# bschrag620/PyRad

Measured on AMD Instinct MI355X. Metric: line*gridpoint evals/sec (whole job), higher is better.
Workload: dtype f64

## Files before the change

### pyrad_amd/csrc/lbl_api.hip

```cpp
#include "../../include/pyrad_hip.h"
#include "lbl_device.h"

#include <algorithm>
#include <chrono>
#include <cmath>
#include <cstdarg>
#include <cstdio>
#include <cstdlib>
#include <cstring>
#include <memory>
#include <mutex>
#include <new>
#include <stdexcept>
#include <string>
#include <type_traits>
#include <vector>


using namespace lbl;
namespace lbl {
void comm_quiesce(lbl_ctx* ctx);
void comm_forget(lbl_ctx* ctx);
}

// ... 17 lines not shown
    DeviceArena cidx;
    DeviceArena work;
    DeviceArena jobs;
    DeviceArena counts;
    DeviceArena bal;
    DeviceArena red;
    DeviceArena zeros;
    size_t zeros_set = 0;
    void* host_stage = nullptr;
    size_t host_stage_cap = 0;
    size_t host_stage_head = 0;
    hipEvent_t stage_ev[2] = {nullptr, nullptr};
    bool stage_ev_set[2] = {false, false};
    struct DescSlot { std::vector<char> bytes; void* dptr = nullptr; size_t cap = 0; };
    DescSlot desc_cache[4];
    int desc_next = 0;
    std::vector<char> desc_build;
    int last_jobs = 0;
    int last_blocks_per_job = 0;
    std::vector<int> last_list_blocks;
    int accum_variant = 5;
    int accum_R = 0;
    int accum_LS = 0;
    int gauss_run = 0;
    int bal_workers[9] = {0, 0, 0, 0, 0, 0, 0, 0, 0};
    struct Schedule {
        std::vector<uint64_t> key; int2* d_list; int total; int32_t* d_tabs; std::vector<size_t> tab_off;
        int xcd_tol = 3;
        int sr_chunks = 1;
        int launch_total = 0;
        int xcd_pack = 1;
        void* d_block = nullptr;
        bool pending = false;
        int R = 0, spans_per_tile = 0, total_spans = 0, xcd_chunks = 32;
        long long far_reach = 0;
        double cost_near = 0, cost_edge = 0, cost_far = 0, cost_fixed = 0;
        std::vector<int32_t> span_first, tile_first;
        int32_t* d_src = nullptr;
        std::vector<size_t> src_off;
        bool merge_pending = false;
    };
    std::vector<std::unique_ptr<Schedule>> schedules;
    int accuracy = 0;
    int sweep_ieee = 0;
    int sched_build = 1;
    DeviceArena sched;
// ... 374 lines not shown
} LBL_GUARD_END(ctx)

extern "C" int lbl_profile_read(lbl_ctx* ctx, int kind, int64_t* launches, double* total_ms) try {
    if (!ctx || !launches || !total_ms) return fail(ctx, LBL_ERR_BAD_ARG, "NULL argument");
    if (kind < 0 || kind >= kProfileKinds) return fail(ctx, LBL_ERR_BAD_ARG, "kind out of range");
    HIP_TRY(ctx, hipStreamSynchronize(ctx->stream));
    double tot = 0.0;
    for (auto& p : ctx->ev_rec[kind]) {
        float ms = 0.f;
        HIP_TRY(ctx, hipEventElapsedTime(&ms, p.first, p.second));
        tot += ms;
    }
    *launches = (int64_t)ctx->ev_rec[kind].size();
    *total_ms = tot;
    return LBL_OK;
} LBL_GUARD_END(ctx)

namespace lbl {
void* comm_prof_begin(lbl_ctx* ctx) { return (void*)prof_begin(ctx, PROF_GATHER); }
void comm_prof_end(lbl_ctx* ctx, void* start) { prof_end(ctx, PROF_GATHER, (hipEvent_t)start); }
}

static uint64_t option_state(const lbl_ctx* c) {
    const long long v[] = {c->accum_variant, c->accum_R, c->accum_LS, c->gauss_run, c->lpt, c->tile_order, c->skew, c->skew_R, c->skew_LS, c->xcd_chunks, c->xcd_pack, c->xcd_tol, c->far_min_H,
                           c->ablate, c->accuracy, c->sweep_ieee, c->sched_build, c->no_fuse ? 1 : 0,
                           c->bal_workers[1], c->bal_workers[2], c->bal_workers[4], c->bal_workers[8]};
    uint64_t h = 1469598103934665603ull;
    for (long long x : v) { h ^= (uint64_t)x; h *= 1099511628211ull; }
    return h;
}
static int set_option_value(lbl_ctx* ctx, const char* key, int value);

extern "C" int lbl_set_option(lbl_ctx* ctx, const char* key, int value) try {
    if (!ctx || !key) return fail(ctx, LBL_ERR_BAD_ARG, "NULL argument");
    const uint64_t before = option_state(ctx);
    const int rc = set_option_value(ctx, key, value);
    if (option_state(ctx) != before) ctx->epoch++;
    return rc;
} LBL_GUARD_END(ctx)

static int set_option_value(lbl_ctx* ctx, const char* key, int value) {
    if (!strcmp(key, "accum_variant")) {
#ifdef LBL_DIAG
        if (value < 0 || value > 5) return fail(ctx, LBL_ERR_BAD_ARG, "accum_variant must be 0..5");
#else
        if (!(value == 0 || value == 3 || value == 5))
            return fail(ctx, LBL_ERR_BAD_ARG, "accum_variant must be 0, 3 or 5 (1, 2 and 4 are superseded comparison kernels: diagnostic builds only)");
// ... 19 lines not shown
    } else if (!strcmp(key, "accum_skew")) {
        if (value < 0 || value > 2) return fail(ctx, LBL_ERR_BAD_ARG, "accum_skew must be 0, 1 or 2");
        ctx->skew = value;
    } else if (!strcmp(key, "accum_skew_points_per_lane")) {
        if (!(value == 1 || value == 2 || value == 4 || value == 8))
            return fail(ctx, LBL_ERR_BAD_ARG, "accum_skew_points_per_lane must be 1, 2, 4 or 8");
        ctx->skew_R = value;
    } else if (!strcmp(key, "accum_xcd_chunks")) {
        if (value < 0 || value > 64) return fail(ctx, LBL_ERR_BAD_ARG, "accum_xcd_chunks must be 0 (auto: 10..32 by the workgroup count) .. 64");
        ctx->xcd_chunks = value;
    } else if (!strcmp(key, "accum_xcd_tolerance")) {
        if (value < -1 || value > 15) return fail(ctx, LBL_ERR_BAD_ARG, "accum_xcd_tolerance must be -1 (off) .. 15 percent");
        ctx->xcd_tol = value;
    } else if (!strcmp(key, "accum_xcd_pack")) {
        if (value < 0 || value > 3) return fail(ctx, LBL_ERR_BAD_ARG, "accum_xcd_pack must be 0..3");
        ctx->xcd_pack = value;
    } else if (!strcmp(key, "accum_skew_line_split")) {
        if (!(value == 0 || value == 1 || value == 2 || value == 4))
            return fail(ctx, LBL_ERR_BAD_ARG, "accum_skew_line_split must be 0 (auto), 1, 2 or 4");
        ctx->skew_LS = value;
    } else if (!strcmp(key, "accum_gauss_run")) {
        if (value != 0 && value != 16 && value != 32) return fail(ctx, LBL_ERR_BAD_ARG, "accum_gauss_run must be 0 (auto), 16 or 32");
        ctx->gauss_run = value;
    } else if (!strcmp(key, "accum_far_min_window")) {
        if (value < 0) return fail(ctx, LBL_ERR_BAD_ARG, "accum_far_min_window must be >= 0");
        ctx->far_min_H = value;
#ifdef LBL_DIAG
    } else if (!strcmp(key, "debug_ablate")) {
        ctx->ablate = value;
#endif
    } else if (!strcmp(key, "accuracy")) {
        if (value < 0 || value > 1) return fail(ctx, LBL_ERR_BAD_ARG, "accuracy must be 0 (exact) or 1 (budget: 1e-9)");
        ctx->accuracy = value;
    } else if (!strcmp(key, "sweep_ieee_divisions")) {
        if (value < 0 || value > 1) return fail(ctx, LBL_ERR_BAD_ARG, "sweep_ieee_divisions must be 0 or 1");
        ctx->sweep_ieee = value;
    } else if (!strcmp(key, "schedule_build")) {
        if (value < 0 || value > 1) return fail(ctx, LBL_ERR_BAD_ARG, "schedule_build must be 0 (host) or 1 (device)");
        ctx->sched_build = value;
    } else if (!strcmp(key, "layer_step_fused")) {
        if (value < 0 || value > 1) return fail(ctx, LBL_ERR_BAD_ARG, "layer_step_fused must be 0 or 1");
        ctx->no_fuse = value == 0;
    } else if (!strcmp(key, "debug_throw")) {
        if (value == 1) throw std::bad_alloc();
        if (value == 2) throw std::runtime_error("debug_throw");
        if (value == 3) { std::vector<double> v; v.reserve(v.max_size() + 1); }
// ... 818 lines not shown
                              sc->far_reach, sc->cost_near, sc->cost_edge, sc->cost_far, sc->cost_fixed,
                              ctx->n_cu > 0 ? ctx->n_cu : 256, sc->d_tabs, (char*)ctx->sched.ptr + jobs_bytes, sc->d_list, ctx->stream,
                              sc->xcd_chunks, sc->xcd_pack != 0, sc->sr_chunks, sc->xcd_tol, sc->xcd_pack == 2 ? 1 : sc->xcd_pack == 3 ? 0 : -1);
        HIP_TRY(ctx, hipGetLastError());
        sc->pending = false;
    }
    if (ctx->chain_pred && !ctx->capturing) HIP_TRY(ctx, hipStreamWaitEvent(ctx->stream, ctx->chain_pred->accum_done, 0));
    for (size_t gi = 0; gi < groups.size(); ++gi) {
        const Group& g = groups[gi];
        ev = prof_begin(ctx, PROF_ACCUM);
        if (balanced) {
            const size_t S = (size_t)group_spans[gi];
            char* base = (char*)ctx->bal.ptr + bal_off[gi];
            SpanRec* spans = (SpanRec*)base;
            unsigned long long* prefix = (unsigned long long*)(base + S * sizeof(SpanRec));
            unsigned int* cnts = (unsigned int*)(base + S * sizeof(SpanRec) + (S + 1) * sizeof(unsigned long long));
            double* slab = (double*)(base + ((S * sizeof(SpanRec) + S * sizeof(unsigned int) + (S + 1) * sizeof(unsigned long long) + 255) & ~(size_t)255));
            launch_accumulate_balanced(da + g.first, g.count, (int)S, g.R, group_workers[gi], spans, cnts, prefix, slab,
                                       ctx->stream);
        } else if (g.variant == 6) {
            launch_accumulate_skew(da + g.first, g.count, g.max_tiles, g.R, g.worklist, g.total_tiles, ctx->stream, g.LS);
        } else {
            launch_accumulate(da + g.first, g.count, g.max_tiles, g.R, g.LS, g.variant, g.worklist, g.total_tiles,
                              ctx->stream, ctx->accuracy, g.grun);
        }
        prof_end(ctx, PROF_ACCUM, ev);
        HIP_TRY(ctx, hipGetLastError());
    }
    if (ctx->accum_done && !ctx->capturing) HIP_TRY(ctx, hipEventRecord(ctx->accum_done, ctx->stream));
    for (int j = 0; j < n_jobs; ++j) {
        if (!needs_regrid(grid[j])) continue;
        ev = prof_begin(ctx, PROF_REGRID);
        launch_regrid((const double*)ctx->work.ptr + work_off[j], grid[j].n_work, out_dev[j], grid[j].n_base,
                      grid[j].range_min, grid[j].range_max, ctx->stream);
        prof_end(ctx, PROF_REGRID, ev);
        HIP_TRY(ctx, hipGetLastError());
    }
    return LBL_OK;
}

extern "C" int lbl_schedule_export(lbl_ctx* ctx, int k, int32_t* list, int64_t list_cap, int32_t* tabs, int64_t tabs_cap,
                                   int64_t* n_items, int64_t* n_tab_ints, int32_t* built_on_device) try {
    if (!ctx || !n_items || !n_tab_ints) return fail(ctx, LBL_ERR_BAD_ARG, "NULL argument");
    if (k < 0 || (size_t)k >= ctx->schedules.size()) return fail(ctx, LBL_ERR_BAD_ARG, "no such schedule (the cache holds %d)", (int)ctx->schedules.size());
    const lbl_ctx::Schedule& S = *ctx->schedules[ctx->schedules.size() - 1 - (size_t)k];
    if (S.pending) return fail(ctx, LBL_ERR_STATE, "the schedule has not been built yet (no accumulate batch has used it)");
    HIP_TRY(ctx, hipStreamSynchronize(ctx->stream));
// ... 867 lines not shown
```

### pyrad_amd/csrc/lbl_device.h

```cpp
#pragma once
#include <hip/hip_runtime.h>
#include <stdint.h>
#include "lbl_launch_shapes.h"

namespace lbl {

constexpr double kB = 1.38064852E-23;
constexpr double cLight = 299792458.0;
constexpr double hPlanck = 6.62607004e-34;
constexpr double kPi = 3.141592653589793;
constexpr double kInvPi = 0.3183098861837907;
constexpr double kInvSqrtPi = 0.5641895835477563;
constexpr double t0 = 296.0;
constexpr double p0 = 1013.25;
constexpr double avo = 6.022140857E23;

struct __attribute__((aligned(32))) HotRec {
    double cf;
    double a2;
    double KL;
    int32_t dgi;
    int32_t flags;
};
struct __attribute__((aligned(32))) ColdRec {
// ... 198 lines not shown
    double table_half, table_rdx;
    long long n_channels;
    int32_t n_rows, n_table;
    int32_t chunk, pad;
};
void launch_ils_convolve(const IlsArgs* d_args, int shape, int n_rows, long long n_channels, hipStream_t s);

struct ColumnArgs {
    const double* trans[kMaxLayers];
    double layer_T[kMaxLayers];
    double r_layer_T[kMaxLayers];
    double pbkT[kMaxLayers], pbk_surface;
    double r_surface_T;
    int32_t n_layers;
    double start, stop, step, pa, pb, surface_T;
    const double* I_in; double* I_out;
    long long n;
    long long first, count;
};

void launch_line_prep(const PrepJob* d_jobs, int n_jobs, int max_lines, hipStream_t s);
void launch_line_quantities(const PrepJob* d_job, int n_lines, long long* index, double* lhw, double* ghw, double* intensity,
                            int32_t* regime, hipStream_t s);
void launch_accumulate(const AccumJob* d_jobs, int n_jobs, int max_tiles, int R, int LS, int variant,
                       const int2* worklist, int total_tiles, hipStream_t s, int budget = 0, int gauss_run = 16);
void launch_accumulate_skew(const AccumJob* d_jobs, int n_jobs, int max_tiles, int R, const int2* worklist, int total_tiles,
                            hipStream_t s, int LS = 1);
void accumulate_far_field_params(int R, int* far_half_spans, double* far_cost, int budget = 0);
int balanced_workers(int R, int n_cu);
void launch_accumulate_balanced(const AccumJob* d_jobs, int n_jobs, int total_spans, int R, int n_workers,
                                SpanRec* spans, unsigned int* counts, unsigned long long* prefix, double* slab,
                                hipStream_t s);
void launch_regrid(const double* work, long long n_work, double* out, long long n_base, double start, double stop,
                   hipStream_t s);
void launch_layer_sweep(const SweepArgs& a, hipStream_t s);
void launch_column_step(const ColumnStepArgs* d_args, long long first, long long count, hipStream_t s, int budget = 0, int kfold = 0);
void launch_column_sweep(const ColumnArgs* d_args, long long n, hipStream_t s, int budget = 0);
void launch_planck(double* out, long long n, double start, double stop, double T, double rT, double pa, double pb, hipStream_t s);
void launch_band_integral(const double* y, long long n, double* partial, double* result, hipStream_t s);
struct SumArgs { const double* in[kMaxIso]; int32_t n_in; double* out; long long n; };
void launch_sum(const SumArgs& a, hipStream_t s);
constexpr int kMaxRanks = 64;
struct CompactArgs { const double* gathered; double* out; long long slot; long long first[kMaxRanks]; long long count[kMaxRanks]; int32_t world; };
void launch_gather_compact(const CompactArgs& a, long long max_count, hipStream_t s);
void launch_optical(const double* trans, long long n, int kind, double* out, hipStream_t s);
void launch_line_survey(const double* nu, const double* sw, int n_lines, double range_min, double resolution,
                        double* out, long long n_base, hipStream_t s);

// ... 2 lines not shown
```

### pyrad_amd/csrc/lbl_kernels.hip

```cpp
#include "lbl_device.h"
#include "lbl_launch_shapes.h"
#include <cstdlib>
#include <type_traits>

namespace lbl {

#ifdef LBL_DIAG
#define LBL_ABLATE(obj, bit) (((obj).ablate & (bit)) != 0)
#else
#define LBL_ABLATE(obj, bit) false
#endif

__device__ __forceinline__ int uniform_i32(int v) { return __builtin_amdgcn_readfirstlane(v); }

typedef const double __attribute__((address_space(4)))* ConstF64;
typedef const int32_t __attribute__((address_space(4)))* ConstI32;

struct Rec {
    double cf, a2, KL, KG, b, q2;
    int32_t ci, dgi, flags;
};

__device__ __forceinline__ Rec load_rec_scalar(const HotRec* hot, const ColdRec* cold, int i, bool want_cold) {
    ConstF64 h = (ConstF64)(unsigned long long)hot + (long long)i * 4;
// ... 396 lines not shown
            const double t = K * S.D[k];
            S.N[k] = fma(S.N[k], den, t);
            S.D[k] *= den;
        }
        if (++S.cnt == S.every) S.flush();
    }
}

template <int R, bool MASKED, int DIV, int GM>
__device__ __forceinline__ void process_lines_scalar(const HotRec* hot, const ColdRec* cold, int i0, int i1, double x0,
                                                     int wlo, int whi, double Hf, WaveAcc<R>& S) {
    for (int i = i0; i < i1; ++i) {
        Rec r = load_rec_scalar(hot, cold, i, false);
        const double d0 = x0 - r.cf;
        lorentz_term<R, MASKED, DIV>(r.a2, r.KL, r.flags, d0, Hf, S);
        const int dist = max(0, max(r.ci - whi, wlo - r.ci));
        if (dist < r.dgi) {
            r = load_rec_scalar(hot, cold, i, true);
            gauss_term<R, GM>(r.KG, r.b, r.q2 >= 0.0, d0, Hf, r.q2, S.acc);
        }
    }
}

__device__ __forceinline__ void wave_line_ranges(const int32_t* __restrict__ cidx, int n_lines, int wlo, int whi, int H,
                                                 int lane, int& iA, int& iB, int& iC, int& iD) {
    const long long tA = (long long)wlo - H, tB = (long long)whi - H;
    const long long tC = (long long)wlo + H + 1, tD = (long long)whi + H + 1;
    const int q = lane >> 4, jj = lane & 15;
    const long long tgt = q == 0 ? tA : q == 1 ? tB : q == 2 ? tC : tD;
    const unsigned long long gmask = 0xFFFFull << (q * 16);
    int lo = 0, hi = n_lines;
    while (__any(hi > lo)) {
        const long long len = (long long)hi - lo;
        const int pos = lo + (int)(((long long)(jj + 1) * len) / 17);
        const bool below = (len > 0) && ((long long)cidx[len > 0 ? pos : 0] < tgt);
        const int k = __popcll(__ballot(below) & gmask);
        if (len > 0) {
            const int p_k = lo + (int)(((long long)(k + 1) * len) / 17);
            const int p_km1 = lo + (int)(((long long)k * len) / 17);
            const int new_lo = k > 0 ? p_km1 + 1 : lo;
            const int new_hi = k < 16 ? p_k : hi;
            lo = new_lo; hi = new_hi;
        }
    }
    iA = __builtin_amdgcn_readlane(lo, 0);
    iB = __builtin_amdgcn_readlane(lo, 16);
    iC = __builtin_amdgcn_readlane(lo, 32);
    iD = __builtin_amdgcn_readlane(lo, 48);
    if (tB >= tC) { iB = iD; iC = iD; }
}

__device__ __forceinline__ void wave_line_ranges_far(const int32_t* __restrict__ cidx, int n_lines, int wlo, int whi, int H,
                                                     long long fl, long long fr, int lane, int& iA, int& iB, int& iC,
                                                     int& iD, int& iF1, int& iF2, int& iN1, int& iN2, long long nl, long long nr) {
    const long long tA = (long long)wlo - H, tB = (long long)whi - H;
    const long long tC = (long long)wlo + H + 1, tD = (long long)whi + H + 1;
    const int q = lane >> 3, jj = lane & 7;
    const long long tgt = q == 0 ? tA : q == 1 ? tB : q == 2 ? tC : q == 3 ? tD : q == 4 ? fl + 1 : q == 5 ? fr : q == 6 ? nl + 1 : nr;
    const unsigned long long gmask = 0xFFull << (q * 8);
    int lo = 0, hi = n_lines;
    while (__any(hi > lo)) {
        const long long len = (long long)hi - lo;
        const int pos = lo + (int)(((long long)(jj + 1) * len) / 9);
        const bool below = (len > 0) && ((long long)cidx[len > 0 ? pos : 0] < tgt);
        const int k = __popcll(__ballot(below) & gmask);
        if (len > 0) {
            const int p_k = lo + (int)(((long long)(k + 1) * len) / 9);
            const int p_km1 = lo + (int)(((long long)k * len) / 9);
            const int new_lo = k > 0 ? p_km1 + 1 : lo;
            const int new_hi = k < 8 ? p_k : hi;
            lo = new_lo; hi = new_hi;
// ... 318 lines not shown
constexpr int FF_NT_MID = 38;
template <int NT> struct LorentzNear { static constexpr int value = NT == FF_NT_MID ? FF_MID : FarThreshold<NT>::value; };

template <int CTRL>
__device__ __forceinline__ double dpp_move_f64(double v) {
    int lo = __double2loint(v), hi = __double2hiint(v);
    lo = __builtin_amdgcn_update_dpp(0, lo, CTRL, 0xf, 0xf, true);
    hi = __builtin_amdgcn_update_dpp(0, hi, CTRL, 0xf, 0xf, true);
    return __hiloint2double(hi, lo);
}

__device__ __forceinline__ double readlane_f64(double v, int l) {
    return __hiloint2double(__builtin_amdgcn_readlane(__double2hiint(v), l), __builtin_amdgcn_readlane(__double2loint(v), l));
}

__device__ __forceinline__ double wave_sum_f64(double v) {
    v += dpp_move_f64<0xB1>(v);
    v += dpp_move_f64<0x4E>(v);
    v += dpp_move_f64<0x141>(v);
    v += dpp_move_f64<0x140>(v);
    return (readlane_f64(v, 0) + readlane_f64(v, 16)) + (readlane_f64(v, 32) + readlane_f64(v, 48));
}

template <int NT>
__device__ __forceinline__ void wave_sum_rows(double (&C)[NT], double* scratch, int lane) {
    const int wr = lane + (lane >> 3);
    const int rd = (lane >> 3) * 72 + (lane & 7) * 9;
#pragma unroll
    for (int base = 0; base < NT; base += 8) {
        __builtin_amdgcn_wave_barrier();
#pragma unroll
        for (int n = 0; n < 8; ++n)
            if (base + n < NT) scratch[n * 72 + wr] = C[base + n];
        __builtin_amdgcn_fence(__ATOMIC_RELEASE, "wavefront");
        __builtin_amdgcn_wave_barrier();
        double t = 0.0;
        if (base + (lane >> 3) < NT) {
            const double* seg = scratch + rd;
            t = ((seg[0] + seg[1]) + (seg[2] + seg[3])) + ((seg[4] + seg[5]) + (seg[6] + seg[7]));
        }
        t += dpp_move_f64<0xB1>(t);
        t += dpp_move_f64<0x4E>(t);
        t += dpp_move_f64<0x141>(t);
#pragma unroll
        for (int n = 0; n < 8; ++n)
            if (base + n < NT) C[base + n] = readlane_f64(t, n * 8);
    }
    __builtin_amdgcn_wave_barrier();
}

template <int NT> struct FarTerms {
    static constexpr bool exact = NT == FF_NT || NT == FF_NT_MID, budget = NT == FF_NT_BUDGET;
    static constexpr int t4 = budget ? 18 : (NT == FF_NT_MID ? FF_NT : NT);
    static constexpr int t8 = exact ? 20 : (budget ? 12 : NT);
    static constexpr int t16 = exact ? 15 : (budget ? 9 : NT);
    static constexpr int t32 = exact ? 12 : (budget ? 7 : NT);
};

template <int N0, int N1, int NT>
__device__ __forceinline__ void series_terms(double al, double bp, double& qa, double& qb, double (&C)[NT]) {
#pragma unroll
    for (int n = N0; n < N1; ++n) {
        const double qn = fma(al, qb, -(bp * qa));
        C[n] += qn;
        if ((n & 1) == 1) asm volatile("" : "+v"(C[n]));
        qa = qb; qb = qn;
    }
}

template <int R, int NT>
__device__ __forceinline__ void far_field_lines(const HotRec* hot, const ColdRec* cold, int m0, int m1, int stride,
                                                double xc, int wlo, int whi, double x0, double Hf, double* lh, double* lc,
                                                int lane, double (&C)[NT], WaveAcc<R>& S, int gx_lo = 0, int gx_hi = 0) {
    typedef double v2f64 __attribute__((ext_vector_type(2)));
    typedef const v2f64 __attribute__((address_space(1)))* GlobalF64x2;
    const GlobalF64x2 gh = (GlobalF64x2)(unsigned long long)hot;
    const GlobalF64x2 gc = (GlobalF64x2)(unsigned long long)cold;
    const double hh = 32.0 * R;
    v2f64 h0 = {0, 1}, h1 = {0, 0};
    if (m0 + lane < m1) {
        const long long r = (long long)(m0 + lane) * 2;
        h0 = gh[r]; h1 = gh[r + 1];
    }
    for (int c0 = m0; c0 < m1; c0 += stride) {
        const bool valid = c0 + lane < m1;
        const v2f64 w0 = h0, w1 = h1;
        if (c0 + stride + lane < m1) {
            const long long r = (long long)(c0 + stride + lane) * 2;
            h0 = gh[r]; h1 = gh[r + 1];
        }
        const int ci = (int)w0.x;
        const int dgi = __double2loint(w1.y), fl = __double2hiint(w1.y);
        const bool gauss = valid && max(0, max(ci - whi, wlo - ci)) < dgi && !(c0 + lane >= gx_lo && c0 + lane < gx_hi);
        const unsigned long long gmask = __ballot(gauss);
        if (gmask) {
            const unsigned long long emask = __ballot((fl & REC_NO_RECUR) != 0);
            v2f64 c0v = {0, 0}, c1v = {0, 0};
            if (gauss) {
                const long long r = (long long)(c0 + lane) * 2;
                c0v = gc[r]; c1v = gc[r + 1];
            }
            __builtin_amdgcn_wave_barrier();
            reinterpret_cast<v2f64*>(lh)[lane * 2] = w0;
            reinterpret_cast<v2f64*>(lh)[lane * 2 + 1] = w1;
            reinterpret_cast<v2f64*>(lc)[lane * 2] = c0v;
            reinterpret_cast<v2f64*>(lc)[lane * 2 + 1] = c1v;
            __builtin_amdgcn_fence(__ATOMIC_RELEASE, "wavefront");
            __builtin_amdgcn_wave_barrier();
            double unused[16];
            chunk_extras<R, 0>(lh, lc, gmask, emask, 0ull, ~0ull, x0, Hf, S, 0ull, 0.0, lane, unused);
            __builtin_amdgcn_wave_barrier();
        }
        const double dl = w0.x - xc;
        const double sq = fma(dl, dl, w0.y);
        double be = __builtin_amdgcn_rcp(sq);
        be = fma(fma(-sq, be, 1.0), be, be);
        be = fma(fma(-sq, be, 1.0), be, be);
        const double al = (dl * (2.0 * hh)) * be;
        const double bp = (hh * hh) * be;
        double qa = (valid ? w1.x : 0.0) * be;
        C[0] += qa;
        double qb = al * qa;
        C[1] += qb;
        const int nv = min(64, m1 - c0);
        const int ca = __builtin_amdgcn_readlane(ci, 0), cb = __builtin_amdgcn_readlane(ci, nv - 1);
        const int dmin2 = min(abs(2 * (ca - wlo) - (64 * R - 1)), abs(2 * (cb - wlo) - (64 * R - 1)));
        typedef FarTerms<NT> FT;
        series_terms<2, FT::t32, NT>(al, bp, qa, qb, C);
        if (dmin2 < 2 * 32 * 32 * R) {
            series_terms<FT::t32, FT::t16, NT>(al, bp, qa, qb, C);
            if (dmin2 < 2 * 16 * 32 * R) {
                series_terms<FT::t16, FT::t8, NT>(al, bp, qa, qb, C);
                if (dmin2 < 2 * 8 * 32 * R) {
                    series_terms<FT::t8, FT::t4, NT>(al, bp, qa, qb, C);
                    if (FT::t4 < NT && dmin2 < 2 * 4 * 32 * R) series_terms<FT::t4, NT, NT>(al, bp, qa, qb, C);
                }
            }
        }
    }
}

template <int R> struct SkewChunk { static constexpr int value = R >= 8 ? 80 : 112; };

__device__ __forceinline__ unsigned int dpp_max_u32(unsigned int v, unsigned int moved) { return v > moved ? v : moved; }

__device__ __forceinline__ unsigned int wave_prefix_max_u32(unsigned int v) {
    v = dpp_max_u32(v, (unsigned int)__builtin_amdgcn_update_dpp(0, (int)v, 0x111, 0xf, 0xf, false));
    v = dpp_max_u32(v, (unsigned int)__builtin_amdgcn_update_dpp(0, (int)v, 0x112, 0xf, 0xf, false));
    v = dpp_max_u32(v, (unsigned int)__builtin_amdgcn_update_dpp(0, (int)v, 0x114, 0xf, 0xf, false));
    v = dpp_max_u32(v, (unsigned int)__builtin_amdgcn_update_dpp(0, (int)v, 0x118, 0xf, 0xf, false));
    v = dpp_max_u32(v, (unsigned int)__builtin_amdgcn_update_dpp(0, (int)v, 0x142, 0xa, 0xf, false));
    v = dpp_max_u32(v, (unsigned int)__builtin_amdgcn_update_dpp(0, (int)v, 0x143, 0xc, 0xf, false));
    return v;
}

template <int R>
__device__ __forceinline__ void skew_counts(const unsigned int* __restrict__ cnt, int lane, int& lo, int& hi) {
    unsigned int m[R];
// ... 242 lines not shown
}


template <int R>
__device__ __forceinline__ void edge_rounds_masked(const HotRec* hot, const ColdRec* cold, int iA, int iB, int iC, int iD, int wlo,
                                                   int whi, double x0, double Hf, double* lh, double* lc, int lane, WaveAcc<R>& S,
                                                   unsigned long long odd) {
    double unused[16];
    while (odd) {
        const int r = __builtin_ctzll(odd);
        odd &= odd - 1;
        for (int side = 0; side < 2; ++side) {
            const int lo = (side ? iC : iA) + 64 * r, end = side ? iD : iB;
            const int hi = min(lo + 64, end);
            if (lo < hi) accumulate_lines<R, 0>(hot, cold, lo, hi, iB, iC, wlo, whi, x0, Hf, lh, lc, lane, S, unused, 64, 1, 0);
        }
    }
    for (int side = 0; side < 2; ++side) {
        const int lo = (side ? iC : iA) + 64 * 64, end = side ? iD : iB;
        if (lo < end) accumulate_lines<R, 0>(hot, cold, lo, end, iB, iC, wlo, whi, x0, Hf, lh, lc, lane, S, unused, 64, 1, 0);
    }
}

template <int R, int LS, int NT = 0, int GRUN = 16>
__global__ __launch_bounds__((LS > 4 ? 64 * LS : 256), (R >= 4 ? (GRUN == 32 ? 3 : 4) : 1))
void xsec_accumulate_lds_kernel(const AccumJob* __restrict__ jobs, const int2* __restrict__ worklist) {
    constexpr bool FF = NT > 0;
    constexpr int NW = LS > 4 ? LS : 4;
    constexpr int PG = NW / LS;
    static_assert(GRUN == 16 || (GRUN == 32 && FF && R == 4 && LS == 1), "32-point Gaussian runs: production shape of the far-field kernel only");
    constexpr int STAGE_MIN = GRUN == 32 ? 4 * 272 : FF ? 576 : 520;
    constexpr int STAGE = (68 * R > STAGE_MIN) ? 68 * R : STAGE_MIN;
    __shared__ double s_stage[NW][STAGE];
    constexpr bool EDGE_SKEW = FF && LS == 1 && R == 4;
    __shared__ unsigned int s_ecnt[EDGE_SKEW ? NW : 1][2][EDGE_SKEW ? 64 * R + 8 : 1];

    int job = blockIdx.y, tile;
    if (worklist) {
        const int2 wk = worklist[blockIdx.x];
        job = wk.x; tile = wk.y;
    } else {
        tile = xcd_tile(blockIdx.x, jobs[job].n_tiles, jobs[job].pad);
    }
    const AccumJob& J = jobs[job];
    const int lane = threadIdx.x & 63;
    const int wave = uniform_i32(threadIdx.x >> 6);
    const int grp = wave / LS, part = wave % LS;
    const int n_end = J.p_end;
    const long long wave_lo_ll = (long long)J.p_begin + (long long)(tile < 0 ? 0 : tile) * (64LL * R * PG) + (long long)grp * (64LL * R);
    const bool active = tile >= 0 && wave_lo_ll < n_end;
    if (LS == 1 && !active) return;
    const int wlo = active ? (int)wave_lo_ll : 0;
    const int whi = active ? min(wlo + 64 * R - 1, n_end - 1) : 0;
    const int H = J.H;
    const int p0 = wlo + lane * R;
    const double x0 = (double)p0;
    const double Hf = (double)H;
    WaveAcc<R> S;
    S.init(J.flush_every);
    double* lh = s_stage[wave];
    double* lc = s_stage[wave] + 256;

    const int32_t* tab = nullptr;
    if (active && J.span_tab) tab = J.span_tab + (size_t)((wlo - J.p_begin) / (64 * R)) * 8;
    if (active && !FF) {
        int iA, iB, iC, iD;
        if (tab) { iA = uniform_i32(tab[0]); iB = uniform_i32(tab[1]); iC = uniform_i32(tab[2]); iD = uniform_i32(tab[3]); }
        else wave_line_ranges(J.cidx, J.n_lines, wlo, whi, H, lane, iA, iB, iC, iD);
        double G[16];
#pragma unroll
        for (int k = 0; k < 16; ++k) G[k] = 0.0;
        accumulate_lines<R, 2>(J.hot, J.cold, iA + part * 64, iD, iB, iC, wlo, whi, x0, Hf, lh, lc, lane, S, G, 64 * LS);
        if (R == 4) gauss_runs_fold<R, 16>(G, s_stage[wave], lane, S.acc);
        S.flush();
    }
    if (active && FF) {
        constexpr int FAR = FarThreshold<NT>::value;
        constexpr int NEAR = LorentzNear<NT>::value;
        static_assert(NEAR == FAR || EDGE_SKEW, "the mid class needs the near walk that knows the Lorentz sub-range");
        const long long fl = (long long)wlo + 32 * R - 1 - (long long)FAR * 32 * R;
        const long long fr = (long long)wlo + 32 * R + (long long)FAR * 32 * R;
        const double xc = (double)wlo + (32.0 * R - 0.5);
        int iA, iB, iC, iD, iF1, iF2, iN1, iN2;
        if (tab) {
            iA = uniform_i32(tab[0]); iB = uniform_i32(tab[1]); iC = uniform_i32(tab[2]); iD = uniform_i32(tab[3]);
            iF1 = uniform_i32(tab[4]); iF2 = uniform_i32(tab[5]);
            iN1 = NEAR < FAR ? uniform_i32(tab[6]) : iF1; iN2 = NEAR < FAR ? uniform_i32(tab[7]) : iF2;
        }
        else {
            wave_line_ranges_far(J.cidx, J.n_lines, wlo, whi, H, fl, fr, lane, iA, iB, iC, iD, iF1, iF2, iN1, iN2,
                                 (long long)wlo + 32 * R - 1 - (long long)FF_MID * 32 * R, (long long)wlo + 32 * R + (long long)FF_MID * 32 * R);
            if (!(NEAR < FAR)) { iN1 = iF1; iN2 = iF2; }
        }
        if (LBL_ABLATE(J, 8)) { iA = iB; iD = iC; }
        const bool any_far = !LBL_ABLATE(J, 256) && (iN1 - iB) + (iC - iN2) > 0;
        const bool edges_done = EDGE_SKEW;
#ifndef LBL_EDGE_SERIES
#define LBL_EDGE_SERIES 1
#endif
        constexpr bool EDGE_SERIES = EDGE_SKEW && LBL_EDGE_SERIES;
        if (edges_done) {
            unsigned int* eL = s_ecnt[EDGE_SKEW ? wave : 0][0];
            unsigned int* eR = s_ecnt[EDGE_SKEW ? wave : 0][1];
            typedef FarTerms<FF ? NT : FF_NT> FT;
            const int dmin = H - 32 * R;
            unsigned long long odd = 0ull;
            const int n_edge = (iB - iA) + (iD - iC);
            const int nte = dmin >= 32 * 32 * R ? FT::t32 : dmin >= 16 * 32 * R ? FT::t16 : FT::t8;
            if (EDGE_SERIES && dmin >= 8 * 32 * R && n_edge * 21 >= 52 * nte + 250)
                series_edges<R>(J.hot, J.cold, iA, iB, iC, iD, wlo, whi, H, x0, Hf, xc, nte, lh, lc, eL, eR, lane, S, odd);
            else
                skew_edges<R>(J.hot, J.cold, iA, iB, iC, iD, wlo, whi, H, x0, Hf, lh, lc, eL, eR, lane, S, odd);
            if (odd || iB - iA > 64 * 64 || iD - iC > 64 * 64)
                edge_rounds_masked<R>(J.hot, J.cold, iA, iB, iC, iD, wlo, whi, x0, Hf, lh, lc, lane, S, odd);
        }
        if (any_far) {
            S.flush();
            constexpr int NTC = FF ? NT : 2;
            double C[NTC];
#pragma unroll
            for (int n = 0; n < NTC; ++n) C[n] = 0.0;
            far_field_lines<R, NTC>(J.hot, J.cold, iB + ((part + 1) % LS) * 64, iN1, 64 * LS, xc, wlo, whi, x0, Hf, lh, lc, lane, C, S, iF1, iF2);
            far_field_lines<R, NTC>(J.hot, J.cold, iN2 + ((part + 2) % LS) * 64, iC, 64 * LS, xc, wlo, whi, x0, Hf, lh, lc, lane, C, S, iF1, iF2);
            wave_sum_rows<NTC>(C, s_stage[wave], lane);
#pragma unroll
            for (int k = 0; k < R; ++k) {
                const double tau = ((x0 + (double)k) - xc) * (1.0 / (32.0 * R));
                double v = C[NTC - 1];
#pragma unroll
                for (int n = NTC - 2; n >= 0; --n) v = fma(v, tau, C[n]);
                S.acc[k] += v;
            }
        }
        double G[GRUN];
#pragma unroll
        for (int k = 0; k < GRUN; ++k) G[k] = 0.0;
        if (LBL_ABLATE(J, 512)) {
        } else if (edges_done) {
            accumulate_lines<R, 1, GRUN>(J.hot, J.cold, iF1, iF2, iB, iC, wlo, whi, x0, Hf, lh, lc, lane, S, G, 64, LS, part, iN1, iN2);
        } else {
            accumulate_lines<R, 1, GRUN>(J.hot, J.cold, iA, any_far ? iB : iD, iB, iC, wlo, whi, x0, Hf, lh, lc, lane, S, G, 64, LS, part);
            if (any_far) {
                accumulate_lines<R, 1, GRUN>(J.hot, J.cold, iF1, iF2, iB, iC, wlo, whi, x0, Hf, lh, lc, lane, S, G, 64, LS, part);
                accumulate_lines<R, 1, GRUN>(J.hot, J.cold, iC, iD, iB, iC, wlo, whi, x0, Hf, lh, lc, lane, S, G, 64, LS, part);
            }
        }
        if (R == 4) gauss_runs_fold<R, GRUN>(G, s_stage[wave], lane, S.acc);
        S.flush();
    }

    double* mine = s_stage[wave];
    __builtin_amdgcn_wave_barrier();
#pragma unroll
    for (int k = 0; k < R; ++k) mine[span_slot(lane * R + k)] = S.acc[k];
    if (LS > 1) __syncthreads();
    else { __builtin_amdgcn_fence(__ATOMIC_RELEASE, "wavefront"); __builtin_amdgcn_wave_barrier(); }
    if (active) {
        double* __restrict__ out = J.out;
        const int w0 = wave - part;
#pragma unroll
        for (int i = 0; i < R; ++i) {
            if (LS > 1 && (i % LS) != part) continue;
            const int o = i * 64 + lane;
            double t = s_stage[w0][span_slot(o)];
            for (int q = 1; q < LS; ++q) t += s_stage[w0 + q][span_slot(o)];
            if (wlo + o < n_end) output_point(J, out, wlo + o, t);
        }
    }
}

template <int R, bool MASKED>
__device__ __forceinline__ void skew_gauss(const double* __restrict__ lh, int cold_off, int sentinel, int g0, int g1,
                                           double x0, double Hf, WaveAcc<R>& S) {
    typedef double v2f64 __attribute__((ext_vector_type(2)));
    const v2f64* rec = reinterpret_cast<const v2f64*>(lh);
    const int len = max(g1 - g0, 0);
    const int T = wave_max_i32(len);
    for (int t = 0; t < T; ++t) {
        const int jc = t < len ? g0 + t : sentinel;
        const v2f64 h0 = rec[jc * 2];
        const double gf = lh[(jc * 2 + 1) * 2 + 1];
        const v2f64 gg = rec[cold_off + jc * 2];
        const double q2 = lh[(cold_off + jc * 2 + 1) * 2];
        const double d0 = x0 - h0.x;
        const bool need = fabs(d0 + 0.5 * (R - 1)) < gf;
        const bool recur = q2 >= 0.0 && R >= 4;
        const bool need_r = need && recur, need_n = need && !recur;
        if (__any(need_r))
            gauss_term<R, 1, MASKED>(need_r ? gg.x : 0.0, need_r ? gg.y : 0.0, true, d0, Hf, need_r ? q2 : 1.0, S.acc);
        if (__any(need_n))
            gauss_term<R, 0, MASKED>(need_n ? gg.x : 0.0, need_n ? gg.y : 0.0, false, d0, Hf, 0.0, S.acc);
// ... 1571 lines not shown
    hipLaunchKernelGGL(line_prep_merged_kernel, grid, dim3(256), 0, s, d_lists, d_jobs);
}

void launch_line_quantities(const PrepJob* d_job, int n_lines, long long* index, double* lhw, double* ghw, double* intensity,
                            int32_t* regime, hipStream_t s) {
    if (n_lines <= 0) return;
    hipLaunchKernelGGL(line_quantities_kernel, dim3((n_lines + 255) / 256), dim3(256), 0, s, d_job, index, lhw, ghw, intensity, regime);
}

template <int R>
static void launch_accum_scalar(const AccumJob* d_jobs, int n_jobs, int max_tiles, int variant, hipStream_t s) {
    dim3 grid(((max_tiles + 7) / 8) * 8, n_jobs);
    switch (variant) {
#ifdef LBL_DIAG
        case 1: hipLaunchKernelGGL((xsec_accumulate_kernel<R, 2, 0>), grid, dim3(256), 0, s, d_jobs); break;
        case 2: hipLaunchKernelGGL((xsec_accumulate_kernel<R, 2, 1>), grid, dim3(256), 0, s, d_jobs); break;
#endif
        default: hipLaunchKernelGGL((xsec_accumulate_kernel<R, 0, 0>), grid, dim3(256), 0, s, d_jobs); break;
    }
}

template <int R, int NT>
static void launch_accum_lds(const AccumJob* d_jobs, int n_jobs, int max_tiles, int LS, const int2* worklist,
                             int total_tiles, hipStream_t s, int gauss_run = 16) {
    dim3 grid(((max_tiles + 7) / 8) * 8, n_jobs);
    if (worklist) {
        if (total_tiles <= 0) return;
        grid = dim3(total_tiles, 1);
    }
#ifdef LBL_DIAG
    static const int pad = getenv("LBL_DIAG_LDS_PAD") ? atoi(getenv("LBL_DIAG_LDS_PAD")) : 0;
#else
    constexpr int pad = 0;
#endif
    switch (LS) {
        case 8: hipLaunchKernelGGL((xsec_accumulate_lds_kernel<R, 8, NT>), grid, dim3(512), pad, s, d_jobs, worklist); break;
        case 4: hipLaunchKernelGGL((xsec_accumulate_lds_kernel<R, 4, NT>), grid, dim3(256), pad, s, d_jobs, worklist); break;
        case 2: hipLaunchKernelGGL((xsec_accumulate_lds_kernel<R, 2, NT>), grid, dim3(256), pad, s, d_jobs, worklist); break;
        default:
            if constexpr (R == 4 && NT > 0) {
                if (gauss_run == 32) {
                    hipLaunchKernelGGL((xsec_accumulate_lds_kernel<4, 1, (NT == FF_NT ? FF_NT_MID : NT), 32>), grid, dim3(256), pad, s, d_jobs, worklist);
                    break;
                }
            }
            hipLaunchKernelGGL((xsec_accumulate_lds_kernel<R, 1, NT>), grid, dim3(256), pad, s, d_jobs, worklist); break;
    }
}

void launch_accumulate_skew(const AccumJob* d_jobs, int n_jobs, int max_tiles, int R, const int2* worklist, int total_tiles,
                            hipStream_t s, int LS) {
    if (n_jobs <= 0 || max_tiles <= 0) return;
    dim3 grid(((max_tiles + 7) / 8) * 8, n_jobs);
    if (worklist) {
        if (total_tiles <= 0) return;
        grid = dim3(total_tiles, 1);
    }
    if (R == 8 && LS == 4) { hipLaunchKernelGGL((xsec_accumulate_skew_kernel<8, 4>), grid, dim3(256), 0, s, d_jobs, worklist); return; }
    if (R == 8 && LS == 2) { hipLaunchKernelGGL((xsec_accumulate_skew_kernel<8, 2>), grid, dim3(256), 0, s, d_jobs, worklist); return; }
    switch (R) {
        case 8: hipLaunchKernelGGL((xsec_accumulate_skew_kernel<8>), grid, dim3(256), 0, s, d_jobs, worklist); break;
        case 2: hipLaunchKernelGGL((xsec_accumulate_skew_kernel<2>), grid, dim3(256), 0, s, d_jobs, worklist); break;
        case 1: hipLaunchKernelGGL((xsec_accumulate_skew_kernel<1>), grid, dim3(256), 0, s, d_jobs, worklist); break;
        default: hipLaunchKernelGGL((xsec_accumulate_skew_kernel<4>), grid, dim3(256), 0, s, d_jobs, worklist); break;
    }
}

void accumulate_far_field_params(int R, int* far_half_spans, double* far_cost, int budget) {
    *far_half_spans = budget ? FF_FAR_BUDGET : FF_FAR;
    *far_cost = (3.0 * 17.0 + 12.0) / 64.0 / (5.0 * R);
}


void launch_accumulate(const AccumJob* d_jobs, int n_jobs, int max_tiles, int R, int LS, int variant,
                       const int2* worklist, int total_tiles, hipStream_t s, int budget, int gauss_run) {
    if (n_jobs <= 0 || max_tiles <= 0) return;
    if (variant >= 5 && budget) {
        switch (R) {
            case 1: launch_accum_lds<1, FF_NT_BUDGET>(d_jobs, n_jobs, max_tiles, LS, worklist, total_tiles, s); break;
            case 2: launch_accum_lds<2, FF_NT_BUDGET>(d_jobs, n_jobs, max_tiles, LS, worklist, total_tiles, s); break;
            case 4: launch_accum_lds<4, FF_NT_BUDGET>(d_jobs, n_jobs, max_tiles, LS, worklist, total_tiles, s, gauss_run); break;
            default: launch_accum_lds<8, FF_NT_BUDGET>(d_jobs, n_jobs, max_tiles, LS, worklist, total_tiles, s); break;
        }
        return;
    }
    if (variant >= 5) {
        switch (R) {
            case 1: launch_accum_lds<1, FF_NT>(d_jobs, n_jobs, max_tiles, LS, worklist, total_tiles, s); break;
            case 2: launch_accum_lds<2, FF_NT>(d_jobs, n_jobs, max_tiles, LS, worklist, total_tiles, s); break;
            case 4: launch_accum_lds<4, FF_NT>(d_jobs, n_jobs, max_tiles, LS, worklist, total_tiles, s, gauss_run); break;
            default: launch_accum_lds<8, FF_NT>(d_jobs, n_jobs, max_tiles, LS, worklist, total_tiles, s); break;
        }
        return;
    }
    if (variant >= 3) {
        switch (R) {
            case 1: launch_accum_lds<1, 0>(d_jobs, n_jobs, max_tiles, LS, worklist, total_tiles, s); break;
            case 2: launch_accum_lds<2, 0>(d_jobs, n_jobs, max_tiles, LS, worklist, total_tiles, s); break;
            case 4: launch_accum_lds<4, 0>(d_jobs, n_jobs, max_tiles, LS, worklist, total_tiles, s); break;
            default: launch_accum_lds<8, 0>(d_jobs, n_jobs, max_tiles, LS, worklist, total_tiles, s); break;
        }
        return;
    }
    switch (R) {
        case 1: launch_accum_scalar<1>(d_jobs, n_jobs, max_tiles, variant, s); break;
        case 2: launch_accum_scalar<2>(d_jobs, n_jobs, max_tiles, variant, s); break;
        case 4: launch_accum_scalar<4>(d_jobs, n_jobs, max_tiles, variant, s); break;
        default: launch_accum_scalar<8>(d_jobs, n_jobs, max_tiles, variant, s); break;
    }
}

void launch_regrid(const double* work, long long n_work, double* out, long long n_base, double start,
                   double stop, hipStream_t s) {
// ... 339 lines not shown
```

Before: 17080 billion.

## Share far-field series across the workgroup tile for distant lines

```diff
diff --git a/pyrad_amd/csrc/lbl_api.hip b/pyrad_amd/csrc/lbl_api.hip
--- a/pyrad_amd/csrc/lbl_api.hip
+++ b/pyrad_amd/csrc/lbl_api.hip
@@ -63,6 +63,7 @@
     int accum_variant = 5;
     int accum_R = 0;
     int accum_LS = 0;
+    int tile_far = 1;
     int gauss_run = 0;
     int bal_workers[9] = {0, 0, 0, 0, 0, 0, 0, 0, 0};
     struct Schedule {
@@ -483,7 +484,7 @@
 }
 
 static uint64_t option_state(const lbl_ctx* c) {
-    const long long v[] = {c->accum_variant, c->accum_R, c->accum_LS, c->gauss_run, c->lpt, c->tile_order, c->skew, c->skew_R, c->skew_LS, c->xcd_chunks, c->xcd_pack, c->xcd_tol, c->far_min_H,
+    const long long v[] = {c->accum_variant, c->accum_R, c->accum_LS, c->gauss_run, c->tile_far, c->lpt, c->tile_order, c->skew, c->skew_R, c->skew_LS, c->xcd_chunks, c->xcd_pack, c->xcd_tol, c->far_min_H,
                            c->ablate, c->accuracy, c->sweep_ieee, c->sched_build, c->no_fuse ? 1 : 0,
                            c->bal_workers[1], c->bal_workers[2], c->bal_workers[4], c->bal_workers[8]};
     uint64_t h = 1469598103934665603ull;
@@ -549,6 +550,9 @@
     } else if (!strcmp(key, "accum_gauss_run")) {
         if (value != 0 && value != 16 && value != 32) return fail(ctx, LBL_ERR_BAD_ARG, "accum_gauss_run must be 0 (auto), 16 or 32");
         ctx->gauss_run = value;
+    } else if (!strcmp(key, "accum_tile_far")) {
+        if (value < 0 || value > 1) return fail(ctx, LBL_ERR_BAD_ARG, "accum_tile_far must be 0 or 1");
+        ctx->tile_far = value;
     } else if (!strcmp(key, "accum_far_min_window")) {
         if (value < 0) return fail(ctx, LBL_ERR_BAD_ARG, "accum_far_min_window must be >= 0");
         ctx->far_min_H = value;
@@ -1413,7 +1417,7 @@
             launch_accumulate_skew(da + g.first, g.count, g.max_tiles, g.R, g.worklist, g.total_tiles, ctx->stream, g.LS);
         } else {
             launch_accumulate(da + g.first, g.count, g.max_tiles, g.R, g.LS, g.variant, g.worklist, g.total_tiles,
-                              ctx->stream, ctx->accuracy, g.grun);
+                              ctx->stream, (ctx->accuracy ? ACCUM_MODE_BUDGET : 0) | (ctx->tile_far ? ACCUM_MODE_TILE_FAR : 0), g.grun);
         }
         prof_end(ctx, PROF_ACCUM, ev);
         HIP_TRY(ctx, hipGetLastError());
diff --git a/pyrad_amd/csrc/lbl_device.h b/pyrad_amd/csrc/lbl_device.h
--- a/pyrad_amd/csrc/lbl_device.h
+++ b/pyrad_amd/csrc/lbl_device.h
@@ -244,8 +244,9 @@
 void launch_line_prep(const PrepJob* d_jobs, int n_jobs, int max_lines, hipStream_t s);
 void launch_line_quantities(const PrepJob* d_job, int n_lines, long long* index, double* lhw, double* ghw, double* intensity,
                             int32_t* regime, hipStream_t s);
+enum : int { ACCUM_MODE_BUDGET = 1, ACCUM_MODE_TILE_FAR = 2 };
 void launch_accumulate(const AccumJob* d_jobs, int n_jobs, int max_tiles, int R, int LS, int variant,
-                       const int2* worklist, int total_tiles, hipStream_t s, int budget = 0, int gauss_run = 16);
+                       const int2* worklist, int total_tiles, hipStream_t s, int mode = 0, int gauss_run = 16);
 void launch_accumulate_skew(const AccumJob* d_jobs, int n_jobs, int max_tiles, int R, const int2* worklist, int total_tiles,
                             hipStream_t s, int LS = 1);
 void accumulate_far_field_params(int R, int* far_half_spans, double* far_cost, int budget = 0);
diff --git a/pyrad_amd/csrc/lbl_kernels.hip b/pyrad_amd/csrc/lbl_kernels.hip
--- a/pyrad_amd/csrc/lbl_kernels.hip
+++ b/pyrad_amd/csrc/lbl_kernels.hip
@@ -442,14 +442,12 @@
     }
 }
 
-__device__ __forceinline__ void wave_line_ranges(const int32_t* __restrict__ cidx, int n_lines, int wlo, int whi, int H,
-                                                 int lane, int& iA, int& iB, int& iC, int& iD) {
-    const long long tA = (long long)wlo - H, tB = (long long)whi - H;
-    const long long tC = (long long)wlo + H + 1, tD = (long long)whi + H + 1;
+__device__ __forceinline__ void wave_lower_bounds4(const int32_t* __restrict__ cidx, int first, int last, long long tA, long long tB,
+                                                   long long tC, long long tD, int lane, int& iA, int& iB, int& iC, int& iD) {
     const int q = lane >> 4, jj = lane & 15;
     const long long tgt = q == 0 ? tA : q == 1 ? tB : q == 2 ? tC : tD;
     const unsigned long long gmask = 0xFFFFull << (q * 16);
-    int lo = 0, hi = n_lines;
+    int lo = first, hi = last;
     while (__any(hi > lo)) {
         const long long len = (long long)hi - lo;
         const int pos = lo + (int)(((long long)(jj + 1) * len) / 17);
@@ -467,6 +465,13 @@
     iB = __builtin_amdgcn_readlane(lo, 16);
     iC = __builtin_amdgcn_readlane(lo, 32);
     iD = __builtin_amdgcn_readlane(lo, 48);
+}
+
+__device__ __forceinline__ void wave_line_ranges(const int32_t* __restrict__ cidx, int n_lines, int wlo, int whi, int H,
+                                                 int lane, int& iA, int& iB, int& iC, int& iD) {
+    const long long tA = (long long)wlo - H, tB = (long long)whi - H;
+    const long long tC = (long long)wlo + H + 1, tD = (long long)whi + H + 1;
+    wave_lower_bounds4(cidx, 0, n_lines, tA, tB, tC, tD, lane, iA, iB, iC, iD);
     if (tB >= tC) { iB = iD; iC = iD; }
 }
 
@@ -831,8 +836,8 @@
     return (readlane_f64(v, 0) + readlane_f64(v, 16)) + (readlane_f64(v, 32) + readlane_f64(v, 48));
 }
 
-template <int NT>
-__device__ __forceinline__ void wave_sum_rows(double (&C)[NT], double* scratch, int lane) {
+template <int NT, bool PARK = false>
+__device__ __forceinline__ void wave_sum_rows(double (&C)[NT], double* scratch, int lane, double* park = nullptr) {
     const int wr = lane + (lane >> 3);
     const int rd = (lane >> 3) * 72 + (lane & 7) * 9;
 #pragma unroll
@@ -851,6 +856,10 @@
         t += dpp_move_f64<0xB1>(t);
         t += dpp_move_f64<0x4E>(t);
         t += dpp_move_f64<0x141>(t);
+        if (PARK) {
+            if ((lane & 7) == 0 && base + (lane >> 3) < NT) park[base + (lane >> 3)] = t;
+            continue;
+        }
 #pragma unroll
         for (int n = 0; n < 8; ++n)
             if (base + n < NT) C[base + n] = readlane_f64(t, n * 8);
@@ -877,36 +886,41 @@
     }
 }
 
-template <int R, int NT>
+template <int R, int NT, int HS = 32 * R, bool TILE = false, bool GAP = false>
 __device__ __forceinline__ void far_field_lines(const HotRec* hot, const ColdRec* cold, int m0, int m1, int stride,
                                                 double xc, int wlo, int whi, double x0, double Hf, double* lh, double* lc,
-                                                int lane, double (&C)[NT], WaveAcc<R>& S, int gx_lo = 0, int gx_hi = 0) {
+                                                int lane, double (&C)[NT], WaveAcc<R>& S, int gx_lo = 0, int gx_hi = 0,
+                                                int gap_at = 0, int gap_len = 0, bool* reach = nullptr) {
+    auto record = [&](int pos) { return GAP ? pos + (pos >= gap_at ? gap_len : 0) : pos; };
     typedef double v2f64 __attribute__((ext_vector_type(2)));
     typedef const v2f64 __attribute__((address_space(1)))* GlobalF64x2;
     const GlobalF64x2 gh = (GlobalF64x2)(unsigned long long)hot;
     const GlobalF64x2 gc = (GlobalF64x2)(unsigned long long)cold;
-    const double hh = 32.0 * R;
+    const double hh = (double)HS;
     v2f64 h0 = {0, 1}, h1 = {0, 0};
     if (m0 + lane < m1) {
-        const long long r = (long long)(m0 + lane) * 2;
+        const long long r = (long long)record(m0 + lane) * 2;
         h0 = gh[r]; h1 = gh[r + 1];
     }
     for (int c0 = m0; c0 < m1; c0 += stride) {
         const bool valid = c0 + lane < m1;
         const v2f64 w0 = h0, w1 = h1;
         if (c0 + stride + lane < m1) {
-            const long long r = (long long)(c0 + stride + lane) * 2;
+            const long long r = (long long)record(c0 + stride + lane) * 2;
             h0 = gh[r]; h1 = gh[r + 1];
         }
         const int ci = (int)w0.x;
         const int dgi = __double2loint(w1.y), fl = __double2hiint(w1.y);
-        const bool gauss = valid && max(0, max(ci - whi, wlo - ci)) < dgi && !(c0 + lane >= gx_lo && c0 + lane < gx_hi);
+        const int me = record(c0 + lane);
+        const bool gauss = valid && max(0, max(ci - whi, wlo - ci)) < dgi && !(me >= gx_lo && me < gx_hi);
         const unsigned long long gmask = __ballot(gauss);
-        if (gmask) {
+        if (TILE) {
+            if (gmask) *reach = true;
+        } else if (gmask) {
             const unsigned long long emask = __ballot((fl & REC_NO_RECUR) != 0);
             v2f64 c0v = {0, 0}, c1v = {0, 0};
             if (gauss) {
-                const long long r = (long long)(c0 + lane) * 2;
+                const long long r = (long long)me * 2;
                 c0v = gc[r]; c1v = gc[r + 1];
             }
             __builtin_amdgcn_wave_barrier();
@@ -933,16 +947,16 @@
         C[1] += qb;
         const int nv = min(64, m1 - c0);
         const int ca = __builtin_amdgcn_readlane(ci, 0), cb = __builtin_amdgcn_readlane(ci, nv - 1);
-        const int dmin2 = min(abs(2 * (ca - wlo) - (64 * R - 1)), abs(2 * (cb - wlo) - (64 * R - 1)));
+        const int dmin2 = min(abs(2 * (ca - wlo) - (2 * HS - 1)), abs(2 * (cb - wlo) - (2 * HS - 1)));
         typedef FarTerms<NT> FT;
         series_terms<2, FT::t32, NT>(al, bp, qa, qb, C);
-        if (dmin2 < 2 * 32 * 32 * R) {
+        if (dmin2 < 2 * 32 * HS) {
             series_terms<FT::t32, FT::t16, NT>(al, bp, qa, qb, C);
-            if (dmin2 < 2 * 16 * 32 * R) {
+            if (dmin2 < 2 * 16 * HS) {
                 series_terms<FT::t16, FT::t8, NT>(al, bp, qa, qb, C);
-                if (dmin2 < 2 * 8 * 32 * R) {
+                if (dmin2 < 2 * 8 * HS) {
                     series_terms<FT::t8, FT::t4, NT>(al, bp, qa, qb, C);
-                    if (FT::t4 < NT && dmin2 < 2 * 4 * 32 * R) series_terms<FT::t4, NT, NT>(al, bp, qa, qb, C);
+                    if (FT::t4 < NT && dmin2 < 2 * 4 * HS) series_terms<FT::t4, NT, NT>(al, bp, qa, qb, C);
                 }
             }
         }
@@ -1231,10 +1245,12 @@
     }
 }
 
-template <int R, int LS, int NT = 0, int GRUN = 16>
-__global__ __launch_bounds__((LS > 4 ? 64 * LS : 256), (R >= 4 ? (GRUN == 32 ? 3 : 4) : 1))
-void xsec_accumulate_lds_kernel(const AccumJob* __restrict__ jobs, const int2* __restrict__ worklist) {
+template <int NT> struct TileFar { static constexpr int value = NT == FF_NT_MID ? 1536 : 2048; };
+
+template <int R, int LS, int NT, int GRUN, bool TF>
+__device__ __forceinline__ void accumulate_lds_body(const AccumJob* __restrict__ jobs, const int2* __restrict__ worklist) {
     constexpr bool FF = NT > 0;
+    static_assert(!TF || (FF && LS == 1 && R == 4), "the tile-far class: production shape of the far-field kernel only");
     constexpr int NW = LS > 4 ? LS : 4;
     constexpr int PG = NW / LS;
     static_assert(GRUN == 16 || (GRUN == 32 && FF && R == 4 && LS == 1), "32-point Gaussian runs: production shape of the far-field kernel only");
@@ -1243,6 +1259,8 @@
     __shared__ double s_stage[NW][STAGE];
     constexpr bool EDGE_SKEW = FF && LS == 1 && R == 4;
     __shared__ unsigned int s_ecnt[EDGE_SKEW ? NW : 1][2][EDGE_SKEW ? 64 * R + 8 : 1];
+    __shared__ double s_tile[TF ? NW : 1][TF ? NT : 1];
+    __shared__ int s_tile_reach[TF ? NW : 1];
 
     int job = blockIdx.y, tile;
     if (worklist) {
@@ -1258,6 +1276,14 @@
     const int n_end = J.p_end;
     const long long wave_lo_ll = (long long)J.p_begin + (long long)(tile < 0 ? 0 : tile) * (64LL * R * PG) + (long long)grp * (64LL * R);
     const bool active = tile >= 0 && wave_lo_ll < n_end;
+    constexpr int T_FAR = TileFar<NT>::value;
+    const bool tile_on = TF && tile >= 0 && J.H >= T_FAR + 16 * 32 * R && !LBL_ABLATE(J, 256);
+    if (TF && tile_on && !active) {
+        if (lane < NT) s_tile[TF ? wave : 0][TF ? lane : 0] = 0.0;
+        if (lane == 0) s_tile_reach[TF ? wave : 0] = 0;
+        __syncthreads();
+        return;
+    }
     if (LS == 1 && !active) return;
     const int wlo = active ? (int)wave_lo_ll : 0;
     const int whi = active ? min(wlo + 64 * R - 1, n_end - 1) : 0;
@@ -1302,7 +1328,54 @@
             if (!(NEAR < FAR)) { iN1 = iF1; iN2 = iF2; }
         }
         if (LBL_ABLATE(J, 8)) { iA = iB; iD = iC; }
-        const bool any_far = !LBL_ABLATE(J, 256) && (iN1 - iB) + (iC - iN2) > 0;
+        int tL0 = iB, tL1 = iB, tR0 = iC, tR1 = iC;
+        if (TF && tile_on) {
+            const long long tl = (long long)J.p_begin + (long long)tile * (64LL * R * PG);
+            const long long th = min(tl + 64LL * R * PG - 1, (long long)n_end - 1);
+            constexpr int HT = 32 * R * PG;
+            wave_lower_bounds4(J.cidx, iB, iC, th - H, tl + HT - T_FAR, tl + HT + T_FAR, tl + H + 1, lane, tL0, tL1, tR0, tR1);
+            tL1 = min(tL1, iN1); tL0 = min(tL0, tL1);
+            tR0 = max(tR0, iN2); tR1 = max(tR1, tR0);
+            const int n_act = (int)min((long long)NW, (n_end - tl + 64 * R - 1) / (64 * R));
+            constexpr int NTC = FF ? NT : 2;
+            double C[NTC];
+#pragma unroll
+            for (int n = 0; n < NTC; ++n) C[n] = 0.0;
+            bool reach = false;
+            const double tc = (double)tl + (HT - 0.5);
+            far_field_lines<R, NTC, HT, true>(J.hot, J.cold, tL0 + wave * 64, tL1, 64 * n_act, tc, (int)tl, (int)tl + 2 * HT - 1, x0, Hf,
+                                              lh, lc, lane, C, S, 0, 0, 0, 0, &reach);
+            far_field_lines<R, NTC, HT, true>(J.hot, J.cold, tR0 + ((wave + 1) % n_act) * 64, tR1, 64 * n_act, tc, (int)tl, (int)tl + 2 * HT - 1,
+                                              x0, Hf, lh, lc, lane, C, S, 0, 0, 0, 0, &reach);
+            wave_sum_rows<NTC, true>(C, s_stage[wave], lane, s_tile[TF ? wave : 0]);
+            if (lane == 0) s_tile_reach[TF ? wave : 0] = reach ? 1 : 0;
+            __syncthreads();
+            int any_reach = 0;
+#pragma unroll
+            for (int w = 0; w < NW; ++w) any_reach |= s_tile_reach[TF ? w : 0];
+            if (uniform_i32(any_reach)) {
+                tL1 = tL0; tR0 = tR1;
+            } else {
+                double t = 0.0;
+                if (lane < NTC) {
+                    t = s_tile[0][TF ? lane : 0];
+#pragma unroll
+                    for (int w = 1; w < NW; ++w) t += s_tile[TF ? w : 0][TF ? lane : 0];
+                }
+#pragma unroll
+                for (int n = 0; n < NTC; ++n) C[n] = readlane_f64(t, n);
+#pragma unroll
+                for (int k = 0; k < R; ++k) {
+                    const double tau = ((x0 + (double)k) - tc) * (1.0 / HT);
+                    double v = C[NTC - 1];
+#pragma unroll
+                    for (int n = NTC - 2; n >= 0; --n) v = fma(v, tau, C[n]);
+                    S.acc[k] += v;
+                }
+            }
+        }
+        const int gapL = tL1 - tL0, gapR = tR1 - tR0;
+        const bool any_far = !LBL_ABLATE(J, 256) && (iN1 - iB - gapL) + (iC - iN2 - gapR) > 0;
         const bool edges_done = EDGE_SKEW;
 #ifndef LBL_EDGE_SERIES
 #define LBL_EDGE_SERIES 1
@@ -1329,8 +1402,10 @@
             double C[NTC];
 #pragma unroll
             for (int n = 0; n < NTC; ++n) C[n] = 0.0;
-            far_field_lines<R, NTC>(J.hot, J.cold, iB + ((part + 1) % LS) * 64, iN1, 64 * LS, xc, wlo, whi, x0, Hf, lh, lc, lane, C, S, iF1, iF2);
-            far_field_lines<R, NTC>(J.hot, J.cold, iN2 + ((part + 2) % LS) * 64, iC, 64 * LS, xc, wlo, whi, x0, Hf, lh, lc, lane, C, S, iF1, iF2);
+            far_field_lines<R, NTC, 32 * R, false, TF>(J.hot, J.cold, iB + ((part + 1) % LS) * 64, iN1 - gapL, 64 * LS, xc, wlo, whi, x0, Hf,
+                                                       lh, lc, lane, C, S, iF1, iF2, tL0, gapL);
+            far_field_lines<R, NTC, 32 * R, false, TF>(J.hot, J.cold, iN2 + ((part + 2) % LS) * 64, iC - gapR, 64 * LS, xc, wlo, whi, x0, Hf,
+                                                       lh, lc, lane, C, S, iF1, iF2, tR0, gapR);
             wave_sum_rows<NTC>(C, s_stage[wave], lane);
 #pragma unroll
             for (int k = 0; k < R; ++k) {
@@ -1376,6 +1451,18 @@
             if (wlo + o < n_end) output_point(J, out, wlo + o, t);
         }
     }
+}
+
+template <int R, int LS, int NT = 0, int GRUN = 16>
+__global__ __launch_bounds__((LS > 4 ? 64 * LS : 256), (R >= 4 ? (GRUN == 32 ? 3 : 4) : 1))
+void xsec_accumulate_lds_kernel(const AccumJob* __restrict__ jobs, const int2* __restrict__ worklist) {
+    accumulate_lds_body<R, LS, NT, GRUN, false>(jobs, worklist);
+}
+
+template <int NT, int GRUN>
+__global__ __launch_bounds__(256, (GRUN == 32 ? 3 : 4))
+void xsec_accumulate_tile_kernel(const AccumJob* __restrict__ jobs, const int2* __restrict__ worklist) {
+    accumulate_lds_body<4, 1, NT, GRUN, true>(jobs, worklist);
 }
 
 template <int R, bool MASKED>
@@ -2993,7 +3080,7 @@
 
 template <int R, int NT>
 static void launch_accum_lds(const AccumJob* d_jobs, int n_jobs, int max_tiles, int LS, const int2* worklist,
-                             int total_tiles, hipStream_t s, int gauss_run = 16) {
+                             int total_tiles, hipStream_t s, int gauss_run = 16, int tile_far = 0) {
     dim3 grid(((max_tiles + 7) / 8) * 8, n_jobs);
     if (worklist) {
         if (total_tiles <= 0) return;
@@ -3010,8 +3097,14 @@
         case 2: hipLaunchKernelGGL((xsec_accumulate_lds_kernel<R, 2, NT>), grid, dim3(256), pad, s, d_jobs, worklist); break;
         default:
             if constexpr (R == 4 && NT > 0) {
+                constexpr int NT32 = NT == FF_NT ? FF_NT_MID : NT;
                 if (gauss_run == 32) {
-                    hipLaunchKernelGGL((xsec_accumulate_lds_kernel<4, 1, (NT == FF_NT ? FF_NT_MID : NT), 32>), grid, dim3(256), pad, s, d_jobs, worklist);
+                    if (tile_far) hipLaunchKernelGGL((xsec_accumulate_tile_kernel<NT32, 32>), grid, dim3(256), pad, s, d_jobs, worklist);
+                    else hipLaunchKernelGGL((xsec_accumulate_lds_kernel<4, 1, NT32, 32>), grid, dim3(256), pad, s, d_jobs, worklist);
+                    break;
+                }
+                if (tile_far) {
+                    hipLaunchKernelGGL((xsec_accumulate_tile_kernel<NT, 16>), grid, dim3(256), pad, s, d_jobs, worklist);
                     break;
                 }
             }
@@ -3044,13 +3137,14 @@
 
 
 void launch_accumulate(const AccumJob* d_jobs, int n_jobs, int max_tiles, int R, int LS, int variant,
-                       const int2* worklist, int total_tiles, hipStream_t s, int budget, int gauss_run) {
+                       const int2* worklist, int total_tiles, hipStream_t s, int mode, int gauss_run) {
     if (n_jobs <= 0 || max_tiles <= 0) return;
+    const int budget = mode & ACCUM_MODE_BUDGET, tile_far = (mode & ACCUM_MODE_TILE_FAR) ? 1 : 0;
     if (variant >= 5 && budget) {
         switch (R) {
             case 1: launch_accum_lds<1, FF_NT_BUDGET>(d_jobs, n_jobs, max_tiles, LS, worklist, total_tiles, s); break;
             case 2: launch_accum_lds<2, FF_NT_BUDGET>(d_jobs, n_jobs, max_tiles, LS, worklist, total_tiles, s); break;
-            case 4: launch_accum_lds<4, FF_NT_BUDGET>(d_jobs, n_jobs, max_tiles, LS, worklist, total_tiles, s, gauss_run); break;
+            case 4: launch_accum_lds<4, FF_NT_BUDGET>(d_jobs, n_jobs, max_tiles, LS, worklist, total_tiles, s, gauss_run, tile_far); break;
             default: launch_accum_lds<8, FF_NT_BUDGET>(d_jobs, n_jobs, max_tiles, LS, worklist, total_tiles, s); break;
         }
         return;
@@ -3059,7 +3153,7 @@
         switch (R) {
             case 1: launch_accum_lds<1, FF_NT>(d_jobs, n_jobs, max_tiles, LS, worklist, total_tiles, s); break;
             case 2: launch_accum_lds<2, FF_NT>(d_jobs, n_jobs, max_tiles, LS, worklist, total_tiles, s); break;
-            case 4: launch_accum_lds<4, FF_NT>(d_jobs, n_jobs, max_tiles, LS, worklist, total_tiles, s, gauss_run); break;
+            case 4: launch_accum_lds<4, FF_NT>(d_jobs, n_jobs, max_tiles, LS, worklist, total_tiles, s, gauss_run, tile_far); break;
             default: launch_accum_lds<8, FF_NT>(d_jobs, n_jobs, max_tiles, LS, worklist, total_tiles, s); break;
         }
         return;
```

After: 16940 billion. About the same (-0.8%).
